# pierre-borie/Benlsip.jl

Hardware: AMD Instinct MI355X
Metric: PCG subproblems/sec + achieved HBM GB/s, dense m=65536 n=4096 fp64 (higher is better)
Workload: dtype f64

## Files before the change

benlsip.jl_amd/csrc/bh_api.hip:

```cpp
#include "../../include/benlsip_hip.h"
#include "bh_cauchy_plan.h"
#include "bh_free_image_plan.h"
#include "bh_gram_ingest_plan.h"
#include "bh_kernels.hip.h"
#include "bh_launch_ahead.h"
#include "bh_options.h"
#include "bh_pcg_plan.h"
#include "bh_step_chain_plan.h"

#include <dlfcn.h>
#include <fcntl.h>
#include <rccl/rccl.h>
#include <sched.h>
#include <sys/mman.h>
#include <unistd.h>

#include <algorithm>
#include <atomic>
#include <chrono>
#include <cmath>
#include <cstdio>
#include <cstdlib>
#include <cstring>
#include <array>
#include <initializer_list>
#include <string>
#include <thread>
#include <tuple>
#include <vector>

using namespace bh;

static uint64_t g_kernel_launches = 0;
static uint64_t g_mask_epoch = 0;
#undef hipLaunchKernelGGL
#define hipLaunchKernelGGL(kernelName, ...) do { ++g_kernel_launches; hipLaunchKernelGGLInternal((kernelName), __VA_ARGS__); } while (0)

namespace {

struct CgWorkspace {
    int64_t n_pad = 0;
    double *w = nullptr, *r = nullptr, *v = nullptr, *p = nullptr, *Hp = nullptr, *g = nullptr, *wl = nullptr, *wu = nullptr;
    double *x = nullptr, *s = nullptr, *xlow = nullptr, *xupp = nullptr;
    double* hw = nullptr;
    double* hwc = nullptr;
    double *p2 = nullptr, *gpart = nullptr, *rvpart = nullptr;
    double *r2 = nullptr, *hpx = nullptr, *hpx_tail = nullptr;
    double* slab = nullptr;
    double* scalars = nullptr;
    CgState* d_state = nullptr;
    volatile unsigned long long* h_mirror = nullptr;
    unsigned long long* d_mirror = nullptr;
    unsigned tag = 0;
    unsigned long long* d_reroute = nullptr;
    unsigned long long reroute_seq = 0;
    double* d_trace = nullptr;
    int64_t trace_cap = 0;
};

struct PeerShm {
    std::atomic<int> arrive;
    std::atomic<int> generation;
    int failed;
    hipIpcMemHandle_t handle[kMaxPeers];
};
struct PeerComm {
    bool active = false;
    bool broken = false;
    void* inbox = nullptr;
    size_t inbox_bytes = 0;
    void* peer_base[kMaxPeers] = {};
    volatile unsigned long long* h_err = nullptr;
    PeerShm* shm = nullptr;
    PeerArgs args{};
};
constexpr int64_t kPeerCap = 1 << 16;
constexpr int kPeerBlkCap = (int)(kPeerCap / (2 * kPeerBlockChunks));
constexpr size_t kPeerSlotBytes = (size_t)2 * kMaxPeers * kPeerCap * sizeof(double);
constexpr size_t kPeerFlagBytes = (size_t)2 * kMaxPeers * kPeerBlkCap * sizeof(unsigned long long);
constexpr size_t kPeerScalBytes = kPeerFlagBytes;

struct AsyncUpload {
    std::thread worker;
    int32_t rc = BH_OK;
    std::string detail;
    hipStream_t s_copy = nullptr, s_xpose = nullptr;
    double* staging[2] = {nullptr, nullptr};
    hipEvent_t copied[2] = {nullptr, nullptr}, freed[2] = {nullptr, nullptr};
    size_t staging_bytes = 0;
    int64_t chunk_cols = 0;
    bool gram = false;
    double gram_mu = 0.0;
    GramIngestPlan gram_plan{};
    hipStream_t s_gram = nullptr;
    double* gram_part = nullptr;
    int64_t gram_part_doubles = 0;
    bool resources() const { return s_copy != nullptr; }
};

struct Ctx : Options {
    bool init = false;
    int device = -1;
    int flags = 0;
    int n_cu = 0;
    hipStream_t own_stream = nullptr;
    hipStream_t stream = nullptr;
    std::string detail;
    StepNotes notes;
    void* rccl_lib = nullptr;
    ncclComm_t comm = nullptr;
    int rank = 0, nranks = 1;
    ncclResult_t (*p_ncclGetUniqueId)(ncclUniqueId*) = nullptr;
    ncclResult_t (*p_ncclCommInitRank)(ncclComm_t*, int, ncclUniqueId, int) = nullptr;
    ncclResult_t (*p_ncclCommDestroy)(ncclComm_t) = nullptr;
    ncclResult_t (*p_ncclAllReduce)(const void*, void*, size_t, ncclDataType_t, ncclRedOp_t, ncclComm_t, hipStream_t) = nullptr;
    const char* (*p_ncclGetErrorString)(ncclResult_t) = nullptr;
    PeerComm peer;
    int comm_path = 0;
    CgWorkspace cg;
    double* scratch_dev = nullptr;
    struct PooledImage { double* ptr; int64_t doubles; };
    std::vector<PooledImage> image_pool;
    int64_t image_pool_hits = 0;
    AsyncUpload* upload_cache = nullptr;
    int64_t h2d_bytes = 0, d2h_bytes = 0, h2d_calls = 0, d2h_calls = 0;
    volatile unsigned long long* mbox_h = nullptr;
    unsigned long long* mbox_d = nullptr;
    unsigned long long mbox_seq = 0;
    double* rbuf = nullptr;
    int64_t rbuf_cap = 0;
    int live_hess = 0;
    bool reform_vlds_attr_set = false;
    bool vlds_attr_set = false;
    bool cgp_vlds_attr_set = false;
    bool trsm_lds_granted = false;
    size_t trsv_lds_granted = 0;
};

// ... 223 lines not shown
    double* gpart = nullptr;
    int gram_slabs = 1;
    int64_t gram_slab_rows = 0;
    bool G_valid = false;
    double G_mu = 0.0;
    int64_t gram_builds = 0;
    double* geq = nullptr;
    int64_t geq_doubles = 0;
    double* Jf = nullptr;
    int64_t Jf_doubles = 0;
    int* fi_map = nullptr;
    int* fi_ops = nullptr;
    std::vector<int32_t> fi_ops_h;
    FreeImageBook fi;
    uint64_t fi_epoch = 0;
    double* Af = nullptr;
    int64_t Af_doubles = 0;
    uint64_t af_epoch = 0;
    double call_bytes = 0.0;
    double timed_bytes = 0.0;
    int64_t timed_n = 0;
};

struct bh_proj {
    int64_t mA = 0, n = 0, ldA = 0;
    double* Ad = nullptr;
    int nfix = 0, mpp = 0;
    bool active_set = false;
    int* fixrank = nullptr;
    int* fixidx = nullptr;
    double* L = nullptr;
    int64_t L_cap = 0;
    bool have_L = false;
    double* M = nullptr;
    double* Lr = nullptr;
    int* info = nullptr;
    double* tpart = nullptr;
    double* W = nullptr;
    bool linv_valid = false;
    int last_cauchy_form = -1;
    int last_cauchy_launches = 0;
    int last_cauchy_passes = 0;
    bool reduced = false;
    bool M_valid = false;
    std::vector<uint64_t> last_chunks;
    int* newidx = nullptr;
    int* counts = nullptr;
    unsigned long long* chunks_dev = nullptr;
    double* tw = nullptr;
    double* rpad = nullptr;
    double* vtmp = nullptr;
    uint64_t mask_epoch = 0;
};

namespace {

int32_t ensure_cg_workspace(int64_t n_pad, int64_t trace_cap) {
    CgWorkspace& c = g_ctx.cg;
    if (c.n_pad < n_pad) {
        double** vecs[] = {&c.w, &c.r, &c.v, &c.p, &c.Hp, &c.s, &c.x, &c.xlow, &c.xupp, &c.g, &c.wl, &c.wu, &c.hw, &c.hwc, &c.p2, &c.gpart, &c.rvpart,
                           &c.r2, &c.hpx, &c.hpx_tail};
        constexpr int NV = 20;
        dev_free(c.slab);
        c.slab = nullptr;
        g_ctx.notes.workspace_gone();
        BH_TRY(dev_alloc(&c.slab, NV * n_pad + 8));
        BH_HIP(hipMemsetAsync(c.slab, 0, (size_t)(NV * n_pad + 8) * sizeof(double), g_ctx.stream));
        for (int i = 0; i < NV; ++i) *vecs[i] = c.slab + (int64_t)i * n_pad;
        c.scalars = c.slab + NV * n_pad;
        c.n_pad = n_pad;
    }
    if (!c.d_state) {
        BH_TRY(dev_alloc(&c.d_state, 1));
        BH_HIP(hipMemsetAsync(c.d_state, 0, sizeof(CgState), g_ctx.stream));
        void* hp = nullptr;
        BH_HIP(hipHostMalloc(&hp, 64, hipHostMallocMapped | hipHostMallocCoherent));
        memset(hp, 0, 64);
        c.h_mirror = reinterpret_cast<volatile unsigned long long*>(hp);
        void* dp = nullptr;
        BH_HIP(hipHostGetDevicePointer(&dp, hp, 0));
        c.d_mirror = reinterpret_cast<unsigned long long*>(dp);
    }
    if (!c.d_reroute) {
        BH_TRY(dev_alloc(&c.d_reroute, 1));
        BH_HIP(hipMemsetAsync(c.d_reroute, 0, sizeof(unsigned long long), g_ctx.stream));
    }
    if (trace_cap > c.trace_cap) {
        dev_free(c.d_trace);
        c.d_trace = nullptr;
        BH_TRY(dev_alloc(&c.d_trace, 4 * trace_cap));
        c.trace_cap = trace_cap;
    }
    return BH_OK;
}

int32_t check_peer_error();
int32_t hess_ready(bh_hess* H);

int32_t wait_mirror(CgWorkspace& c, unsigned tag, int target, MirrorWord* out, int iter_target = 0) {
    const auto t0 = std::chrono::steady_clock::now();
    unsigned long long spins = 0;
    auto reached = [&](unsigned long long w, MirrorWord* m) {
        if (((w >> 48) & 0xffffu) != (tag & 0xffffu)) return false;
        m->status = (int)((w >> 44) & 0xf);
        m->done = (int)((w >> 40) & 0xf);
        m->iter = (int)((w >> 20) & 0xfffff);
        m->n_hmul = (int)(w & 0xfffff);
        return m->done != 0 || m->n_hmul >= target || (iter_target > 0 && m->iter >= iter_target);
    };
    while (true) {
        if (reached(*c.h_mirror, out)) return BH_OK;
        __builtin_ia32_pause();
        if ((++spins & 0xffff) == 0) {
            if (g_ctx.peer.active && *g_ctx.peer.h_err != 0ull) return check_peer_error();
            hipError_t q = hipStreamQuery(g_ctx.stream);
            if (q != hipSuccess && q != hipErrorNotReady) return fail(BH_ERR_HIP, std::string("CG loop: ") + hipGetErrorString(q));
            if (q == hipSuccess) {
                MirrorWord m2{};
                if (!reached(*c.h_mirror, &m2)) return fail(BH_ERR_HIP, "internal: stream drained but the loop state did not reach the launch target");
                continue;
            }
            if (std::chrono::steady_clock::now() - t0 > std::chrono::seconds(120))
                return fail(BH_ERR_HIP, "CG loop: no progress for 120 s", false);
        }
    }
}

bool comm_active() { return g_ctx.comm != nullptr || g_ctx.peer.active; }
bool use_peer_path() { return g_ctx.peer.active && (g_ctx.comm_path == 1 || g_ctx.comm == nullptr); }

int32_t allreduce_inplace(double* buf, int64_t count, bh_hess* H, const CgState* state = nullptr) {
    if (!comm_active() || count <= 0) return BH_OK;
    if (use_peer_path()) {
        for (int64_t off = 0; off < count; off += kPeerCap) {
            const int nch = (int)((std::min(kPeerCap, count - off) + 1) / 2);
            hipLaunchKernelGGL(reduce_exchange_kernel, dim3((nch + kPeerBlockChunks - 1) / kPeerBlockChunks), dim3(256), 0, g_ctx.stream,
                               (const double*)nullptr, (int64_t)0, nch, 0, buf + off, state, g_ctx.peer.args);
        }
        BH_HIP(hipGetLastError());
    } else {
        BH_NCCL(g_ctx.p_ncclAllReduce(buf, buf, (size_t)count, ncclDouble, ncclSum, g_ctx.comm, g_ctx.stream));
    }
    if (H) H->stats.n_allreduce += 1;
    return BH_OK;
}

int32_t check_peer_error() {
    if (g_ctx.peer.active && g_ctx.peer.h_err != nullptr && *g_ctx.peer.h_err != 0ull)
        return fail(BH_ERR_RCCL, "peer-buffer all-reduce: a rank did not arrive within the timeout (exchange #" +
                                     std::to_string(*g_ctx.peer.h_err) + "); results are invalid", false);
    return BH_OK;
}

int32_t reduce_slabs(bh_hess* H, int grid, double* z_out, const CgState* state) {
    const int nblk = (H->nchunks + kPeerBlockChunks - 1) / kPeerBlockChunks;
    if (use_peer_path() && nblk <= kPeerBlkCap) {
        hipLaunchKernelGGL(reduce_exchange_kernel, dim3(nblk), dim3(256), 0, g_ctx.stream, (const double*)H->partials, H->ld, H->nchunks,
                           grid, z_out, state, g_ctx.peer.args);
        BH_HIP(hipGetLastError());
        H->stats.n_allreduce += 1;
        return BH_OK;
    }
    hipLaunchKernelGGL(reduce_partials_kernel, dim3(nblk), dim3(256), 0, g_ctx.stream, H->partials, H->ld, H->nchunks, grid, z_out, state);
    BH_HIP(hipGetLastError());
    return allreduce_inplace(z_out, H->n, H, state);
}

constexpr int kPanelChunks = 2048;
// ... 1769 lines not shown
    in.hw_wanted = hw_wanted; in.hw_free_part_ok = hw_wanted && hw_free_part_ok; in.atol_f2b_positive = atol_f2b > 0; in.allow_free_image = allow_free_image;
    in.free_image_eq = g_ctx.opt_free_image_eq;
    p.sel = pcg_select(in);
    const int batch = launch_batch_size(H);
    const bool rccl_path = comm_active() && !use_peer_path();
    int cold = std::min(batch, rccl_path ? 1 : 2);
    p.sched.max_units = max_iter; p.sched.batch = batch; p.sched.off = 0; p.sched.look_first = true;
    p.sched.await_iter = false; p.sched.lock_step = true;
    p.pbuf[0] = c.p; p.pbuf[1] = c.p2;
    if (p.sel.shape == PCG_FUSED) {
        p.nrows = p.gram ? H->ld : H->d + H->q_eff;
        pcg_fused_geometry(p, H->nchunks, (int)n);
        p.vv_off = (int)(n_pad / 4);
        p.rvbuf[0] = c.rvpart; p.rvbuf[1] = c.rvpart + n_pad / 2;
        p.sched.await_iter = true; p.sched.lock_step = p.sel.rccl_gen;
        cold = p.sel.rccl_gen ? 1 : std::min(batch, 2);
    } else if (p.sel.shape == PCG_RCCL_BOX) {
        p.nrows = H->d + H->q_eff;
        p.cfg = rs_cfg; p.grid = grid_for(rs_cfg, p.nrows); p.nblk = (H->nchunks + 15) / 16;
        p.rbuf[0] = c.r; p.rbuf[1] = c.r2;
        p.gbuf[0] = H->sq_partials + H->g_cap; p.gbuf[1] = H->sq_partials + 2 * (int64_t)H->g_cap;
        cold = 1;
    }
    p.sched.first = launch_ahead_first(H->last_n_hmul, cold);
    return p;
}

static void pcg_use_free_image(PcgRun& r) {
    bh_hess* H = r.H; CgWorkspace& c = r.c;
    const FreeImageBook& b = H->fi;
    r.fi_use = true;
    r.og = c.x; r.owl = c.xlow; r.owu = c.xupp; r.ow = c.s;
    r.ofix = nullptr;
    if (r.hw != nullptr) r.hw = c.hwc;
    r.on = (int)b.nfree; r.onch = (int)(round_up(b.nfree, 16) / 2);
    r.old = b.ldf;
    pcg_fused_geometry(r.plan, r.onch, r.on);
    H->call_bytes = free_image_bytes(H);
    c.reroute_seq += 1;
}

static void pcg_compact_proj_args(ProjArgs& pa, const PcgRun& r) {
    pa.A = r.H->Af; pa.ldA = r.old; pa.n = r.on; pa.nfix = 0; pa.fixrank = nullptr; pa.nch_pad = r.onch;
}

static int32_t pcg_fused_stream(PcgRun& r, int j) {
    bh_hess* H = r.H; CgWorkspace& c = r.c; const PcgPlan& p = r.plan;
    RowStreamArgs ra = rs_args(H, p.nrows, nullptr);
    ra.partials = H->partials;
    if (p.gram) { ra.J = H->G; ra.d_rows = p.nrows; ra.mu = 1.0; ra.partials = nullptr; ra.t_out = c.Hp; }
    if (r.fi_use) { ra.J = H->Jf; ra.ld = r.old; ra.nchunks = r.onch; }
    if (p.sel.fuse_gen) { ra.v = c.p; ra.negate = 0; }
    else { ra.v = r.og; ra.negate = 1; ra.negmask = r.ofix; }
    CgFuse& f = ra.cf;
    f.st = c.d_state; f.j = j; f.n = r.on; f.max_iter = p.max_iter; f.init_done = p.sel.gen_linv ? 2 : p.sel.fuse_gen ? 1 : 0; f.vv_off = p.vv_off;
    f.vvec = c.v; f.p_old = p.pbuf[(j - 1) & 1]; f.p_new = p.pbuf[j & 1];
    f.rvpart = p.rvbuf[(j - 1) & 1]; f.nrv = p.nrv;
    f.w = r.ow; f.wl = r.owl; f.wu = r.owu;
    if (r.fi_use) { f.reroute = c.d_reroute; f.reroute_seq = c.reroute_seq; }
    f.sqpart = H->sq_partials; f.gpart = H->sq_partials + H->g_cap;
    f.kappa2 = r.a.kappa2; f.atol_f2b = r.a.atol_f2b;
    f.trace = r.a.trace; f.trace_cap = r.a.trace_cap; f.mirror = r.a.mirror; f.tag = r.a.tag;
    int slot = -1;
    const bool expect_stop = j == r.expect_stop_at || j > p.max_iter || (r.expect_stop_at == 0 && j > 1);
    BH_TRY(profile_begin(H, j - 1, &slot));
    if (p.gram) launch_gram_cg(p.cfg, ra, p.grid, r.s, expect_stop);
    else launch_row_stream_cgp(p.cfg, ra, p.grid, r.s, expect_stop);
    if (slot >= 0) BH_HIP(hipEventRecord(H->ev[2 * slot + 1], r.s));
    return BH_OK;
}

static int32_t pcg_fused_update(PcgRun& r, int j) {
    bh_hess* H = r.H; bh_proj* P = r.P; CgWorkspace& c = r.c; const PcgPlan& p = r.plan; hipStream_t s = r.s;
    const int nblk = p.nblk, grid = p.grid;
    CgUpdArgs u{};
    u.st = c.d_state; u.j = j; u.partials = H->partials; u.ld = r.old; u.nchunks = r.onch; u.G = grid; u.Gs = grid; u.Gq = grid;
    u.sqpart = H->sq_partials; u.gpart = H->sq_partials + H->g_cap; u.rvpart_in = p.rvbuf[(j - 1) & 1]; u.rvpart_out = p.rvbuf[j & 1]; u.nrv = p.nrv;
    u.p = p.pbuf[j & 1]; u.w = r.ow; u.hw = r.hw; u.r = c.r; u.g = r.og; u.v = c.v; u.fixrank = r.ofix;
    if (r.fi_use) { u.map = H->fi_map; u.w_full = r.wp; u.reroute = c.d_reroute; u.reroute_seq = c.reroute_seq; }
    u.n = r.on; u.atol_neg = r.a.atol_neg; u.trace = r.a.trace; u.trace_cap = r.a.trace_cap; u.mirror = r.a.mirror; u.tag = r.a.tag;
    if (p.gram) { u.partials = c.Hp; u.Gs = 1; }
    if (!p.sel.fuse_gen) {
        if (p.sel.peer_fused) hipLaunchKernelGGL((cg_reduce_update_kernel<false, true>), dim3(nblk), dim3(256), 0, s, u, g_ctx.peer.args);
        else hipLaunchKernelGGL((cg_reduce_update_kernel<false, false>), dim3(nblk), dim3(256), 0, s, u, PeerArgs{});
        return BH_OK;
    }
    if (p.sel.rccl_gen) {
        const int n_pad = r.a.n_pad;
        hipLaunchKernelGGL(reduce_partials_sq_kernel, dim3(nblk), dim3(256), 0, s, (const double*)H->partials, H->ld, H->nchunks, grid,
                           c.hpx, (const double*)H->sq_partials, n_pad, (const CgState*)c.d_state, j);
        BH_HIP(hipGetLastError());
        BH_TRY(allreduce_inplace(c.hpx, (int64_t)n_pad + 2, H));
        u.partials = c.hpx; u.Gs = 1; u.sqpart = c.hpx + n_pad; u.Gq = 1;
    }
    u.A = P->Ad; u.ldA = P->ldA; u.mA = (int)P->mA; u.tpart = P->tpart; u.init_in_memory = p.sel.gen_linv ? 0 : 1;
    if (r.fi_use) { u.A = H->Af; u.ldA = r.old; }
    if (r.fi_use) hipLaunchKernelGGL(cg_reduce_update_compact_kernel, dim3(nblk), dim3(256), 0, s, u);
    else if (p.sel.peer_fused) hipLaunchKernelGGL((cg_reduce_update_kernel<true, true>), dim3(nblk), dim3(256), 0, s, u, g_ctx.peer.args);
    else hipLaunchKernelGGL((cg_reduce_update_kernel<true, false>), dim3(nblk), dim3(256), 0, s, u, PeerArgs{});
    ProjArgs pa = proj_args(P, c.d_state, true);
    pa.tpart = P->tpart; pa.tpart_nblk = nblk; pa.rvpart = p.rvbuf[j & 1]; pa.fused_j = j;
    if (p.sel.gen_linv) {
        pa.W = P->W; pa.nch_pad = r.onch; pa.Mgram = p.sel.linv_refine ? P->M : nullptr;
        if (r.fi_use) pcg_compact_proj_args(pa, r);
        hipLaunchKernelGGL((proj_apply_linv_kernel<false>), dim3((unsigned)p.nrv), dim3(256), 0, s, pa, (const double*)c.r, c.v);
        return BH_OK;
    }
    hipLaunchKernelGGL(trsv_small_kernel, dim3(1), dim3(256), 0, s, pa);
    hipLaunchKernelGGL((proj_left_mul_tr_kernel<true, 4>), dim3((p.nch_v + 63) / 64), dim3(256), 0, s, pa, (const double*)c.r, c.v);
    return BH_OK;
}

static int32_t pcg_fused_first(PcgRun& r) {
    bh_hess* H = r.H; bh_proj* P = r.P; CgWorkspace& c = r.c; const PcgPlan& p = r.plan; hipStream_t s = r.s;
    if (r.fi_use) {
        FreeGatherArgs ga{};
        ga.g = r.a.g; ga.wl = r.a.wl; ga.wu = r.a.wu; ga.fixrank = P->fixrank; ga.map = H->fi_map;
        ga.gc = c.x; ga.wlc = c.xlow; ga.wuc = c.xupp; ga.wc = c.s; ga.w = r.wp;
        ga.n = r.a.n; ga.n_pad = r.a.n_pad; ga.nfree = r.on;
        ga.reroute = c.d_reroute; ga.seq = c.reroute_seq; ga.mirror = r.a.mirror; ga.tag = r.a.tag;
        hipLaunchKernelGGL(free_image_gather_kernel, dim3((unsigned)((r.a.n_pad + 255) / 256)), dim3(256), 0, s, ga);
    }
    if (p.sel.gen_linv) {
        if (!P->linv_valid) {
            hipLaunchKernelGGL(tri_inv_small_kernel, dim3(1), dim3(256), 0, s, (const double*)P->Lr, (int)P->mA, P->W);
            P->linv_valid = true;
        }
        ProjArgs pa = proj_args(P, nullptr, true);
        if (r.fi_use) pcg_compact_proj_args(pa, r);
        hipLaunchKernelGGL(proj_left_mul_kernel, dim3((unsigned)P->mA), dim3(256), 0, s, pa, r.og);
        pa.tpart = P->tw; pa.tpart_nblk = 1; pa.rvpart = p.rvbuf[0]; pa.vvpart = p.rvbuf[0] + p.vv_off; pa.p_out = c.p;
        pa.W = P->W; pa.nch_pad = r.onch; pa.Mgram = p.sel.linv_refine ? P->M : nullptr; pa.fused_j = 0;
        hipLaunchKernelGGL((proj_apply_linv_kernel<true>), dim3((unsigned)p.nrv), dim3(256), 0, s, pa, r.og, c.v);
    } else if (p.sel.fuse_gen) {
        hipLaunchKernelGGL((cg_init_kernel<false>), dim3(1), dim3(CG_T), 0, s, r.a);
        BH_TRY(launch_project(P, c.r, c.v, c.d_state));
        hipLaunchKernelGGL(cg_init_finish_kernel, dim3(1), dim3(CG_T), 0, s, r.a);
    }
    return pcg_fused_stream(r, 1);
}

static int32_t pcg_fused_unit(PcgRun& r, int index) {
    BH_TRY(pcg_fused_update(r, index + 1));
    BH_TRY(pcg_fused_stream(r, index + 2));
    BH_HIP(hipGetLastError());
    return BH_OK;
}

static int32_t pcg_rccl_box_stream(PcgRun& r, int j) {
    bh_hess* H = r.H; CgWorkspace& c = r.c; const PcgPlan& p = r.plan; const CgArgs& a = r.a;
    RowStreamArgs ra = rs_args(H, p.nrows, nullptr);
    ra.partials = H->partials;
    ra.v = a.g; ra.negate = 1; ra.negmask = a.fixrank;
    CgFuse& f = ra.cf;
    f.st = c.d_state; f.j = j; f.n = a.n; f.max_iter = p.max_iter; f.init_done = 0;
    f.p_old = p.pbuf[(j - 1) & 1]; f.p_new = p.pbuf[j & 1];
    f.r_old = p.rbuf[(j - 1) & 1]; f.r_new = p.rbuf[j & 1];
    f.gpart_in = p.gbuf[(j - 1) & 1]; f.gpart = p.gbuf[j & 1];
    f.w_rw = r.wp; f.w = r.wp; f.hw = r.hw; f.g = a.g; f.fixrank = a.fixrank;
    f.wl = a.wl; f.wu = a.wu;
    f.sqpart = H->sq_partials;
    f.Hp = c.hpx; f.sq_index = a.n_pad;
    f.kappa2 = a.kappa2; f.atol_f2b = a.atol_f2b; f.atol_neg = a.atol_neg;
    f.trace = a.trace; f.trace_cap = a.trace_cap; f.mirror = a.mirror; f.tag = a.tag;
    int slot = -1;
    BH_TRY(profile_begin(H, j - 1, &slot));
    launch_row_stream_cgp3(p.cfg, ra, p.grid, r.s);
// ... 28 lines not shown
    bh_hess* H = r.H; CgWorkspace& c = r.c;
    if (r.plan.sel.fold_init && index == 0) {
        BH_TRY(launch_hmul(H, r.a.g, c.Hp, nullptr, index, true, r.a.fixrank));
        launch_cg_first_step(r.a, r.s);
        return BH_OK;
    }
    BH_TRY(launch_hmul(H, c.p, c.Hp, c.d_state, index));
    if (r.P->mA == 0) {
        launch_cg_step<0>(r.a, r.s);
    } else {
        launch_cg_step<1>(r.a, r.s);
        BH_TRY(launch_project(r.P, c.r, c.v, c.d_state));
        launch_cg_step<2>(r.a, r.s);
    }
    return BH_OK;
}

static int32_t pcg_launch_first(PcgRun& r) {
    switch (r.plan.sel.shape) {
        case PCG_FUSED: return pcg_fused_first(r);
        case PCG_RCCL_BOX: return pcg_rccl_box_stream(r, 1);
        default: return pcg_separate_first(r);
    }
}
static int32_t pcg_launch_unit(PcgRun& r, int index) {
    switch (r.plan.sel.shape) {
        case PCG_FUSED: return pcg_fused_unit(r, index);
        case PCG_RCCL_BOX: return pcg_rccl_box_unit(r, index);
        default: return pcg_separate_unit(r, index);
    }
}

static int32_t pcg_run(bh_hess* H, bh_proj* P, const double* gp, const double* wlp, const double* wup, double* wp, bool w_in_ws,
                       double kappa2, double atol_negcurv, double atol_f2b, int64_t trace_cap, PcgFin* fin_out, double* hw = nullptr,
                       bool g_pad_zeroed = false ,
                       bool allow_free_image = true ,
                       bool hw_free_part_ok = false ) {
    const int64_t n = H->n, n_pad = H->ld;
    const int64_t max_iter64 = 2 * (n - P->mA - P->nfix);
    if (max_iter64 < 0) return fail(BH_ERR_PRECONDITION, "n - mA - count(fixvars) < 0");
    if (max_iter64 >= 0xfffff) return fail(BH_ERR_UNSUPPORTED, "2*(n - mA - count(fixvars)) exceeds the 20-bit iteration counters of the progress word");
    CgWorkspace& c = g_ctx.cg;
    H->ev_pending.clear();
    g_ctx.notes.cg_loop_begins(hw != nullptr);
    H->call_bytes = hmul_bytes(H);

    PcgRun run{H, P, c, g_ctx.stream};
    CgArgs& a = run.a;
    a.st = c.d_state; a.w = wp; a.r = c.r; a.v = c.v; a.p = c.p; a.Hp = c.Hp; a.g = gp; a.wl = wlp; a.wu = wup;
    a.fixrank = P->nfix > 0 ? P->fixrank : nullptr;
    a.n = (int)n; a.n_pad = (int)n_pad; a.w_in_ws = w_in_ws ? 1 : 0; a.max_iter = (int)max_iter64; a.kappa2 = kappa2; a.atol_neg = atol_negcurv; a.atol_f2b = atol_f2b;
    a.trace = trace_cap > 0 ? c.d_trace : nullptr; a.trace_cap = (int)std::min<int64_t>(trace_cap, 0x7fffffff);
    a.mirror = c.d_mirror; a.tag = next_mirror_tag(c);
    a.hw = hw;
    run.wp = wp; run.hw = hw;
    run.og = gp; run.owl = wlp; run.owu = wup; run.ow = wp; run.ofix = a.fixrank;
    run.on = (int)n; run.onch = H->nchunks; run.old = H->ld;
    run.expect_stop_at = H->last_n_hmul > 0 ? H->last_n_hmul + 1 : 0;

    run.plan = pcg_make_plan(H, P, a.max_iter, gp == c.g || n == n_pad, hw != nullptr, hw_free_part_ok, atol_f2b, allow_free_image);
    const PcgSelection& sel = run.plan.sel;
    if (sel.shape != PCG_SEPARATE) BH_TRY(hess_ready(H));
    if (sel.shape == PCG_FUSED && run.plan.gram) BH_TRY(ensure_gram(H));
    H->stats.cg_kernels = sel.cg_kernels;
    if (sel.shape != PCG_SEPARATE || sel.fold_init) BH_TRY(zero_staged_g_padding(c, gp, n, n_pad, g_pad_zeroed));
    bool fi_use = false, fi_earns = false;
    if (sel.free_image_eligible) BH_TRY(free_image_prepare(H, P, &fi_use, &fi_earns));
    if (fi_use && P->mA > 0) {
        BH_TRY(free_image_prepare_lineq(H, P, &fi_use));
        if (!fi_use) H->fi.served -= 1;
    }
    if (fi_use) pcg_use_free_image(run);

    BH_TRY(pcg_launch_first(run));
    MirrorWord mw{};
    BH_TRY(launch_ahead(run.plan.sched, [&](int index) { return pcg_launch_unit(run, index); },
                        [&](int n_hmul_target, int iter_target, MirrorWord* m) { return wait_mirror(c, a.tag, n_hmul_target, m, iter_target); }, &mw));
    if (!mw.done) return fail(BH_ERR_HIP, "internal: CG loop did not terminate");
    if (fi_use && mw.status == kCgReroute) {
        H->fi.served -= 1;
        return pcg_run(H, P, gp, wlp, wup, wp, w_in_ws, kappa2, atol_negcurv, atol_f2b, trace_cap, fin_out, hw, g_pad_zeroed, false);
    }
    if (fi_earns) H->fi.credit += free_image_saving(mw.n_hmul, P->nfix, n);
    const bool results_final = sel.shape == PCG_FUSED && !sel.rccl_gen &&
                               (mw.status == BH_CG_SOLVED || mw.status == BH_CG_MAX_ITER_REACHED || mw.status == BH_CG_NONE);
    pcg_fin_fill(fin_out, mw, a.tag, results_final);
    fin_out->compact = fi_use;
    if (sel.peer_fused) H->stats.n_allreduce += mw.n_hmul;
    return BH_OK;
}

static void read_tie_words(bh_hess* H) {
    const unsigned long long tw = g_ctx.cg.h_mirror[1], mb = g_ctx.cg.h_mirror[2];
    H->margin_kind = (int)((tw >> 48) & 0xf); H->tie_flags = (int)((tw >> 40) & 0xff);
    H->tie_first = (int)((tw >> 20) & 0xfffff); H->margin_at = (int)(tw & 0xfffff);
    memcpy(&H->min_margin, &mb, sizeof(double));
    H->tie_read = true;
}

static int32_t pcg_finish(bh_hess* H, const PcgFin& fin, bool drained = true) {
    if (!fin.done) return fail(BH_ERR_HIP, "internal: CG loop did not terminate");
    H->stats.n_pcg += 1;
    H->last_n_hmul = fin.n_hmul;
    H->tie_tag = fin.tag;
    H->tie_read = false;
    if (drained) read_tie_words(H);
    H->stats.n_hmul += fin.n_hmul;
    H->stats.n_cg_iter += fin.iter - 1;
    H->stats.n_proj += fin.iter;
    if (!H->ev_pending.empty()) {
        for (size_t i = 0; i < H->ev_pending.size(); ++i) {
            if (H->ev_pending[i] >= fin.n_hmul) continue;
            float ms = 0.f;
            if (hipEventElapsedTime(&ms, H->ev[2 * i], H->ev[2 * i + 1]) == hipSuccess) {
                H->stats.hmul_ms += ms;
                H->stats.hmul_timed += 1;
                H->timed_bytes += H->call_bytes;
                H->timed_n += 1;
            }
        }
        if (H->timed_n > 0) H->stats.bytes_per_hmul = H->timed_bytes / (double)H->timed_n;
        H->ev_pending.clear();
    }
    return BH_OK;
}

static int32_t pcg_impl(bh_hess* H, bh_proj* P, const double* g_minor, const double* w_l, const double* w_u, double kappa2,
                        double atol_negcurv, double atol_f2b, double* w_out, int32_t* status, int32_t* iters, double* trace,
                        int64_t trace_cap, int32_t* n_hmul_out, bool dev) {
    BH_REQUIRE_INIT();
    if (!H) return fail(BH_ERR_INVALID_ARG, "NULL bh_hess");
    BH_TRY(check_proj_ready(P));
    if (!g_minor || !w_l || !w_u || !w_out) return fail(BH_ERR_INVALID_ARG, "NULL vector argument");
    if (H->n != P->n) return fail(BH_ERR_SHAPE, "H.n != lincons.n");
    if (trace == nullptr) trace_cap = 0;
    if (trace_cap < 0) return fail(BH_ERR_INVALID_ARG, "negative trace_cap");
    const int64_t n = H->n;
    BH_TRY(ensure_cg_workspace(H->ld, trace_cap));
    CgWorkspace& c = g_ctx.cg;
    auto aligned16 = [](const void* q) { return (reinterpret_cast<uintptr_t>(q) & 15u) == 0; };
    const bool in_place = dev && (n % 2 == 0) && aligned16(g_minor) && aligned16(w_l) && aligned16(w_u) && aligned16(w_out) &&
                          (!comm_active() || n == H->ld);
    const double *gp = g_minor, *wlp = w_l, *wup = w_u;
    double* wp = w_out;
    if (!in_place) {
        if (!dev) {
            BH_TRY(stage_vecs(c.g, {g_minor, w_l, w_u}, n, c.n_pad));
        } else {
            BH_TRY(stage_vec(c.g, g_minor, n, true));
            BH_TRY(stage_vec(c.wl, w_l, n, true));
            BH_TRY(stage_vec(c.wu, w_u, n, true));
        }
        gp = c.g; wlp = c.wl; wup = c.wu; wp = c.w;
    }
    PcgFin fin{};
    BH_TRY(pcg_run(H, P, gp, wlp, wup, wp, !in_place, kappa2, atol_negcurv, atol_f2b, trace_cap, &fin, nullptr, !dev));
    if (!in_place) BH_TRY(fetch_vec(w_out, c.w, n, dev));
    if (trace_cap > 0) count_d2h((size_t)4 * trace_cap * sizeof(double));
    if (trace_cap > 0) note_dma();
    if (trace_cap > 0) BH_HIP(hipMemcpyAsync(trace, c.d_trace, (size_t)4 * trace_cap * sizeof(double), hipMemcpyDeviceToHost, g_ctx.stream));
    const bool drain = g_ctx.opt_final_sync || !(in_place && trace_cap == 0 && fin.results_final);
    if (drain) BH_TRY(sync_flush());
    BH_TRY(pcg_finish(H, fin, drain));
    if (status) *status = fin.status;
    if (iters) *iters = fin.iter;
    if (n_hmul_out) *n_hmul_out = fin.n_hmul;
    return BH_OK;
}
// ... 1053 lines not shown
```

benlsip.jl_amd/csrc/bh_cgfuse.hip.h:

```cpp
#pragma once
#include <hip/hip_runtime.h>
#include <stdint.h>
#include "bh_reduce.hip.h"
#include "bh_cg.hip.h"
#include "bh_comm.hip.h"

namespace bh {

struct CgUpdArgs {
    CgState* st;
    int j;
    const double* partials; int64_t ld; int nchunks; int G;
    int Gs, Gq;
    const double* sqpart;
    const double* gpart;
    const double* rvpart_in;
    double* rvpart_out;
    int nrv;
    const double* p;
    double* w; double* hw;
    double* r; const double* g;
    double* v;
    const int* fixrank;
    int n;
    double atol_neg;
    double* trace; int trace_cap;
    unsigned long long* mirror; unsigned tag;
    const double* A; int64_t ldA; int mA;
    double* tpart;
    int init_in_memory;
    const int* map; double* w_full;
    const unsigned long long* reroute; unsigned long long reroute_seq;
};

template <bool GEN, bool PEER>
__global__ __launch_bounds__(256) void cg_reduce_update_kernel(CgUpdArgs a, PeerArgs pa) {
    constexpr bool SCAT = !GEN;
#include "bh_cgfuse_body.hip.h"
}

__global__ __launch_bounds__(256) void cg_reduce_update_compact_kernel(CgUpdArgs a) {
    constexpr bool GEN = true, PEER = false, SCAT = true;
    const PeerArgs pa{};
#include "bh_cgfuse_body.hip.h"
}

}
```

benlsip.jl_amd/csrc/bh_cgfuse_body.hip.h:

```cpp
    CgState* st = a.st;
    if (st->stop_at != 0 && a.j > st->stop_at) return;
    if (a.reroute != nullptr && *a.reroute == a.reroute_seq) return;
    __shared__ double2 sm[16][17];
    __shared__ double rvs[16];
    __shared__ double2 rsm[16];
    const int tid = threadIdx.x, cl = tid & 15, rl = tid >> 4;
    const int c = blockIdx.x * 16 + cl;
    const bool valid = c < a.nchunks;
    const int64_t ld2 = a.ld >> 1;
    const double QNAN = __longlong_as_double(0x7ff8000000000000ll);

    const bool upd = (rl == 0) && valid;
    const bool from_g = (a.j == 1 && !a.init_in_memory);
    double2 pk = make_double2(0.0, 0.0), wk = pk, hwk = pk, rk = pk;
    int2 fr = make_int2(-1, -1);
    if (upd) {
        pk = reinterpret_cast<const double2*>(a.p)[c];
        if (from_g) {
            rk = reinterpret_cast<const double2*>(a.g)[c];
        } else {
            rk = reinterpret_cast<const double2*>(a.r)[c];
            wk = reinterpret_cast<const double2*>(a.w)[c];
            if (a.hw != nullptr) hwk = reinterpret_cast<const double2*>(a.hw)[c];
        }
    }
    TieRegs tr;
    tr.load(st);
    const int max_iter = st->max_iter;
    const double rtv_state = st->rtv;
    LaneBatch<8> b_sq, b_gp, b_rv;
    b_sq.issue(a.sqpart, a.Gq);
    b_gp.issue(a.gpart, a.G);
    b_rv.issue(a.rvpart_in, a.nrv);
    const double2* P2 = reinterpret_cast<const double2*>(a.partials);
    const int cc = min(c, a.nchunks - 1);
    SlabBatch sb;
    sb.issue(P2, ld2, cc, rl, a.Gs);
    double2 arow[4];
    if (GEN) {
        const double2* A2 = reinterpret_cast<const double2*>(a.A);
        const int64_t ldA2 = a.ldA >> 1;
#pragma unroll
        for (int k = 0; k < 4; ++k) arow[k] = A2[(int64_t)min(rl + 16 * k, a.mA - 1) * ldA2 + cc];
    }
    int2 mp = make_int2(-1, -1);
    if (SCAT && upd && a.map != nullptr) mp = reinterpret_cast<const int2*>(a.map)[c];
    if (upd && a.fixrank != nullptr) fr = reinterpret_cast<const int2*>(a.fixrank)[c];

    const double2 acc = sb.fold(P2, ld2, cc, rl, a.Gs);
    sm[rl][cl] = acc;

    double pHp = wave_sum(b_sq.fold_sum(a.sqpart, a.Gq));
    if (PEER) {
        __shared__ int s_timeout;
        __shared__ double2 xs[kMaxPeers][16];
        __shared__ double ps[kMaxPeers];
        if (tid == 0) s_timeout = 0;
        __syncthreads();
        if (rl == 0) {
            double2 t = sm[0][cl];
#pragma unroll
            for (int q = 1; q < 16; ++q) { t.x += sm[q][cl].x; t.y += sm[q][cl].y; }
            sm[15][cl] = t;
        }
        __syncthreads();
        const double2 mine = sm[15][cl];
        const unsigned long long seq = *pa.seq;
        const int par = (int)(seq & 1ull);
        const int64_t slot = ((int64_t)par * kMaxPeers + pa.rank) * pa.cap;
        const int64_t fidx = ((int64_t)par * kMaxPeers + pa.rank) * pa.nblk_cap + blockIdx.x;
        if (rl < pa.nranks && valid) sys_store_f64x2(pa.slots[rl] + slot + 2 * (int64_t)c, mine);
        if (rl < pa.nranks && cl == 0) __hip_atomic_store(pa.scal[rl] + fidx, pHp, __ATOMIC_RELAXED, __HIP_MEMORY_SCOPE_SYSTEM);
        asm volatile("s_waitcnt vmcnt(0)" ::: "memory");
        __syncthreads();
        if (rl < pa.nranks && cl == 0) __hip_atomic_store(pa.flags[rl] + fidx, seq, __ATOMIC_RELAXED, __HIP_MEMORY_SCOPE_SYSTEM);
        if (rl < pa.nranks && cl == 0) {
            const unsigned long long* f = pa.flags[pa.rank] + ((int64_t)par * kMaxPeers + rl) * pa.nblk_cap + blockIdx.x;
            const unsigned long long t0 = wall_clock64();
            const bool dead = __hip_atomic_load(pa.dead, __ATOMIC_RELAXED, __HIP_MEMORY_SCOPE_AGENT) != 0u;
            if (dead) s_timeout = 1;
            while (!dead && __hip_atomic_load(f, __ATOMIC_RELAXED, __HIP_MEMORY_SCOPE_SYSTEM) != seq) {
                __builtin_amdgcn_s_sleep(8);
                if (wall_clock64() - t0 > pa.timeout_ticks) {
                    s_timeout = 1;
                    __hip_atomic_store(pa.err, seq, __ATOMIC_RELAXED, __HIP_MEMORY_SCOPE_SYSTEM);
                    __hip_atomic_store(pa.dead, 1u, __ATOMIC_RELAXED, __HIP_MEMORY_SCOPE_AGENT);
                    break;
                }
            }
        }
        asm volatile("" ::: "memory");
        __syncthreads();
        if (rl < pa.nranks) {
            double2 got = make_double2(0.0, 0.0);
            if (valid) got = sys_load_f64x2(pa.slots[pa.rank] + ((int64_t)par * kMaxPeers + rl) * pa.cap + 2 * (int64_t)c);
            xs[rl][cl] = got;
            if (cl == 0) ps[rl] = __hip_atomic_load(pa.scal[pa.rank] + ((int64_t)par * kMaxPeers + rl) * pa.nblk_cap + blockIdx.x,
                                                  __ATOMIC_RELAXED, __HIP_MEMORY_SCOPE_SYSTEM);
        }
        __syncthreads();
        double2 t = xs[0][cl];
        double ph = ps[0];
        for (int r = 1; r < pa.nranks; ++r) { t.x += xs[r][cl].x; t.y += xs[r][cl].y; ph += ps[r]; }
        if (s_timeout) { ph = __longlong_as_double(0x7ff8000000000000ll); }
        pHp = ph;
        __syncthreads();
        sm[rl][cl] = (rl == 0) ? t : make_double2(0.0, 0.0);
        if (tid == 0) {
            const unsigned done = atomicAdd(pa.arrive, 1u) + 1u;
            if (done == gridDim.x) { *pa.arrive = 0u; *pa.seq = seq + 1ull; }
        }
    }
    const double gamma = wave_min(b_gp.fold_min(a.gpart, a.G));
    const double rtv = (a.j == 1) ? rtv_state : wave_sum(b_rv.fold_sum(a.rvpart_in, a.nrv));
    int cont = 0, neg = 0, outside = 0;
    double step = 0.0, alpha = QNAN;
    bool add_w = true;
    if (pHp <= a.atol_neg) {
        neg = 1;
        if (fabs(pHp) > a.atol_neg) step = gamma;
        else add_w = false;
    } else {
        alpha = __ddiv_rn(rtv, pHp);
        outside = alpha > gamma;
        if (outside) step = gamma;
        else { step = alpha; cont = 1; }
    }
    __syncthreads();

    double rv_part = 0.0;
    if (rl == 0 && valid) {
        double2 hp = sm[0][cl];
#pragma unroll
        for (int q = 1; q < 16; ++q) { hp.x += sm[q][cl].x; hp.y += sm[q][cl].y; }
        const bool e0 = 2 * c < a.n, e1 = 2 * c + 1 < a.n;
        if (add_w) {
            wk.x = __dadd_rn(wk.x, __dmul_rn(step, pk.x));
            wk.y = __dadd_rn(wk.y, __dmul_rn(step, pk.y));
            hwk.x = __dadd_rn(hwk.x, __dmul_rn(step, hp.x));
            hwk.y = __dadd_rn(hwk.y, __dmul_rn(step, hp.y));
        }
        double2 vk = make_double2(0.0, 0.0);
        if (cont) {
            rk.x = __dadd_rn(rk.x, __dmul_rn(alpha, hp.x));
            rk.y = __dadd_rn(rk.y, __dmul_rn(alpha, hp.y));
            vk.x = (fr.x >= 0) ? 0.0 : rk.x;
            vk.y = (fr.y >= 0) ? 0.0 : rk.y;
        }
        if (!e0) { wk.x = 0.0; hwk.x = 0.0; rk.x = 0.0; vk.x = 0.0; }
        if (!e1) { wk.y = 0.0; hwk.y = 0.0; rk.y = 0.0; vk.y = 0.0; }
        if (cont && !GEN) rv_part = fma(rk.y, vk.y, rk.x * vk.x);
        if (add_w || a.j == 1) {
            reinterpret_cast<double2*>(a.w)[c] = wk;
            if (a.hw != nullptr) reinterpret_cast<double2*>(a.hw)[c] = hwk;
            if (SCAT && mp.x >= 0) a.w_full[mp.x] = wk.x;
            if (SCAT && mp.y >= 0) a.w_full[mp.y] = wk.y;
        }
        if (cont || a.j == 1) {
            reinterpret_cast<double2*>(a.r)[c] = rk;
            if (!GEN) reinterpret_cast<double2*>(a.v)[c] = vk;
        }
        if (GEN) rsm[cl] = vk;
    } else if (GEN && rl == 0) {
        rsm[cl] = make_double2(0.0, 0.0);
    }
    if (!GEN) {
        if (rl == 0) rvs[cl] = rv_part;
        __syncthreads();
        if (tid == 0) {
            double t = 0.0;
#pragma unroll
            for (int q = 0; q < 16; ++q) t += rvs[q];
            a.rvpart_out[blockIdx.x] = t;
        }
    } else {
        __syncthreads();
        if (cont) {
            const double2 rm = rsm[cl];
#pragma unroll
            for (int k = 0; k < 4; ++k) {
                const int i = rl + 16 * k;
                if (i < a.mA) {
                    double prod = valid ? fma(arow[k].y, rm.y, arow[k].x * rm.x) : 0.0;
                    prod = row16_sum(prod);
                    if (cl == 0) a.tpart[(int64_t)blockIdx.x * a.mA + i] = prod;
                }
            }
        }
    }

    if (blockIdx.x == 0 && tid == 0) {
        st->pHp = pHp; st->gamma = gamma; st->alpha = alpha; st->n_hmul = a.j; st->rtv = rtv;
        st->neg_curvature = neg; st->outside_region = outside; st->need_proj = 0; st->iter = a.j;
        tr.note_step_a(pHp, a.atol_neg, alpha, gamma, a.j);
        tr.store(st);
        if (a.trace != nullptr && a.j <= a.trace_cap) {
            double* row = a.trace + 4 * (int64_t)(a.j - 1);
            row[0] = pHp; row[1] = alpha; row[2] = (neg && !add_w) ? QNAN : gamma; row[3] = rtv;
        }
        int status = 4;
        if (!cont) {
            status = cg_status_of(0, outside, neg, a.j, max_iter);
            st->approx_solved = 0; st->done = 1; st->stop_at = a.j;
            st->status = status;
        }
        publish_word(a.mirror, a.tag, status, cont ? 0 : 1, a.j, a.j, tr);
    }
```

benlsip.jl_amd/csrc/bh_pcg_plan.h:

```cpp
#pragma once
#include <cstdint>

namespace bh {

enum PcgShape : int {
    PCG_SEPARATE = 0,
    PCG_FUSED = 1,
    PCG_RCCL_BOX = 2,
};

struct PcgSelectIn {
    int64_t mA;
    bool gram_handle;
    int64_t cg_fused, gram_cg_fused, linv_refine, fold_init;
    bool comm, peer_path;
    bool reduced;
    bool tpart, W, M_valid;
    bool lda_is_ld;
    bool rs_cfg_ok;
    bool cgp3_ok;
    bool peer_blocks_fit;
    bool iterates;
    bool g_padded;
    bool vectors_in_regs;
    bool hw_wanted;
    bool atol_f2b_positive;
    bool allow_free_image;
    bool hw_free_part_ok;
    int64_t free_image_eq;
};

struct PcgSelection {
    PcgShape shape;
    bool fuse_gen;
    bool gen_linv;
    bool linv_refine;
    bool peer_fused;
    bool rccl_gen;
    bool free_image_eligible;
    bool fold_init;
    int cg_kernels;
};

inline PcgSelection pcg_select(const PcgSelectIn& in) {
    PcgSelection o{};
    const bool box = in.mA == 0;
    const int64_t cg_fused = !in.gram_handle ? in.cg_fused : (in.gram_cg_fused != 0 && !in.comm) ? 1 : 0;
    const bool fuse_gen = !box && cg_fused >= 1 && in.reduced && in.mA <= 64 && in.tpart && in.lda_is_ld && (!in.gram_handle || in.W);
    const bool gen_linv = fuse_gen && cg_fused == 1 && in.W;
    const bool peer_fused = in.comm && in.peer_path && (box || fuse_gen) && in.peer_blocks_fit;
    const bool rccl_gen = in.comm && !in.peer_path && fuse_gen;
    const bool feasible = in.rs_cfg_ok && in.iterates && in.g_padded;
    if ((box || fuse_gen) && cg_fused != 0 && feasible && (!in.comm || peer_fused || rccl_gen)) {
        o.shape = PCG_FUSED;
        o.fuse_gen = fuse_gen; o.gen_linv = gen_linv; o.peer_fused = peer_fused; o.rccl_gen = rccl_gen;
        o.linv_refine = gen_linv && in.linv_refine != 0 && in.M_valid && in.mA >= 2;
        o.cg_kernels = (box ? 2 : gen_linv ? 3 : 4) + (rccl_gen ? 1 : 0);
        o.free_image_eligible = in.allow_free_image && box && !in.gram_handle && !in.comm && (!in.hw_wanted || in.hw_free_part_ok) &&
                                in.atol_f2b_positive;
        if (in.free_image_eq != 0 && gen_linv && !in.gram_handle && !in.comm && !in.hw_wanted && in.atol_f2b_positive && in.allow_free_image)
            o.free_image_eligible = true;
        return o;
    }
    if (!in.gram_handle && in.comm && !in.peer_path && box && in.cg_fused != 0 && feasible && in.cgp3_ok) {
        o.shape = PCG_RCCL_BOX;
        o.cg_kernels = 2;
        return o;
    }
    o.shape = PCG_SEPARATE;
    o.fold_init = box && in.vectors_in_regs && in.fold_init != 0 && feasible;
    return o;
}

}
```

Before: 1778.

## Decide CG stop verdict in last-arriving block of fused update kernel

```diff
diff --git a/benlsip.jl_amd/csrc/bh_api.hip b/benlsip.jl_amd/csrc/bh_api.hip
--- a/benlsip.jl_amd/csrc/bh_api.hip
+++ b/benlsip.jl_amd/csrc/bh_api.hip
@@ -54,6 +54,7 @@
     unsigned tag = 0;
     unsigned long long* d_reroute = nullptr;
     unsigned long long reroute_seq = 0;
+    unsigned* d_arrive = nullptr;
     double* d_trace = nullptr;
     int64_t trace_cap = 0;
 };
@@ -443,8 +444,9 @@
         c.d_mirror = reinterpret_cast<unsigned long long*>(dp);
     }
     if (!c.d_reroute) {
-        BH_TRY(dev_alloc(&c.d_reroute, 1));
-        BH_HIP(hipMemsetAsync(c.d_reroute, 0, sizeof(unsigned long long), g_ctx.stream));
+        BH_TRY(dev_alloc(&c.d_reroute, 16));
+        BH_HIP(hipMemsetAsync(c.d_reroute, 0, 16 * sizeof(unsigned long long), g_ctx.stream));
+        c.d_arrive = reinterpret_cast<unsigned*>(c.d_reroute + 8);
     }
     if (trace_cap > c.trace_cap) {
         dev_free(c.d_trace);
@@ -2380,7 +2382,10 @@
     if (p.gram) { u.partials = c.Hp; u.Gs = 1; }
     if (!p.sel.fuse_gen) {
         if (p.sel.peer_fused) hipLaunchKernelGGL((cg_reduce_update_kernel<false, true>), dim3(nblk), dim3(256), 0, s, u, g_ctx.peer.args);
-        else hipLaunchKernelGGL((cg_reduce_update_kernel<false, false>), dim3(nblk), dim3(256), 0, s, u, PeerArgs{});
+        else {
+            u.arrive = c.d_arrive; u.verdict = pcg_update_takes_verdict(j, r.expect_stop_at, p.max_iter, p.gram) ? 1 : 0;
+            hipLaunchKernelGGL((cg_reduce_update_kernel<false, false>), dim3(nblk), dim3(256), 0, s, u, PeerArgs{});
+        }
         return BH_OK;
     }
     if (p.sel.rccl_gen) {
@@ -2575,8 +2580,9 @@
         return pcg_run(H, P, gp, wlp, wup, wp, w_in_ws, kappa2, atol_negcurv, atol_f2b, trace_cap, fin_out, hw, g_pad_zeroed, false);
     }
     if (fi_earns) H->fi.credit += free_image_saving(mw.n_hmul, P->nfix, n);
+    const bool ticket = sel.shape == PCG_FUSED && !sel.fuse_gen && !sel.peer_fused;
     const bool results_final = sel.shape == PCG_FUSED && !sel.rccl_gen &&
-                               (mw.status == BH_CG_SOLVED || mw.status == BH_CG_MAX_ITER_REACHED || mw.status == BH_CG_NONE);
+                               (ticket || mw.status == BH_CG_SOLVED || mw.status == BH_CG_MAX_ITER_REACHED || mw.status == BH_CG_NONE);
     pcg_fin_fill(fin_out, mw, a.tag, results_final);
     fin_out->compact = fi_use;
     if (sel.peer_fused) H->stats.n_allreduce += mw.n_hmul;
diff --git a/benlsip.jl_amd/csrc/bh_cgfuse.hip.h b/benlsip.jl_amd/csrc/bh_cgfuse.hip.h
--- a/benlsip.jl_amd/csrc/bh_cgfuse.hip.h
+++ b/benlsip.jl_amd/csrc/bh_cgfuse.hip.h
@@ -31,6 +31,7 @@
     int init_in_memory;
     const int* map; double* w_full;
     const unsigned long long* reroute; unsigned long long reroute_seq;
+    unsigned* arrive; int verdict;
 };
 
 template <bool GEN, bool PEER>
diff --git a/benlsip.jl_amd/csrc/bh_cgfuse_body.hip.h b/benlsip.jl_amd/csrc/bh_cgfuse_body.hip.h
--- a/benlsip.jl_amd/csrc/bh_cgfuse_body.hip.h
+++ b/benlsip.jl_amd/csrc/bh_cgfuse_body.hip.h
@@ -28,6 +28,8 @@
     tr.load(st);
     const int max_iter = st->max_iter;
     const double rtv_state = st->rtv;
+    double tol_cg = 0.0;
+    if constexpr (!GEN && !PEER) tol_cg = st->tol_cg;
     LaneBatch<8> b_sq, b_gp, b_rv;
     b_sq.issue(a.sqpart, a.Gq);
     b_gp.issue(a.gpart, a.G);
@@ -189,14 +191,41 @@
         }
     }
 
-    if (blockIdx.x == 0 && tid == 0) {
+    bool commit = blockIdx.x == 0 && tid == 0;
+    bool vstop = false, vsolved = false;
+    double rtv_next = 0.0;
+    if constexpr (!GEN && !PEER) {
+        if (!cont || a.verdict) {
+            __shared__ int s_last;
+            asm volatile("s_waitcnt vmcnt(0)" ::: "memory");
+            __syncthreads();
+            if (tid == 0) {
+                __builtin_amdgcn_fence(__ATOMIC_RELEASE, "agent");
+                asm volatile("s_waitcnt vmcnt(0)" ::: "memory");
+                s_last = __hip_atomic_fetch_add(a.arrive, 1u, __ATOMIC_RELAXED, __HIP_MEMORY_SCOPE_AGENT) == gridDim.x - 1u;
+            }
+            __syncthreads();
+            if (!s_last || tid >= 64) return;
+            __builtin_amdgcn_fence(__ATOMIC_ACQUIRE, "agent");
+            commit = tid == 0;
+            if (commit) __hip_atomic_store(a.arrive, 0u, __ATOMIC_RELAXED, __HIP_MEMORY_SCOPE_AGENT);
+            if (cont) {
+                rtv_next = wave_fixed_sum(a.rvpart_out, (int)gridDim.x);
+                vsolved = fabs(rtv_next) < tol_cg;
+                vstop = vsolved || a.j + 1 > max_iter;
+            }
+        }
+    }
+    if (commit) {
         st->pHp = pHp; st->gamma = gamma; st->alpha = alpha; st->n_hmul = a.j; st->rtv = rtv;
         st->neg_curvature = neg; st->outside_region = outside; st->need_proj = 0; st->iter = a.j;
         tr.note_step_a(pHp, a.atol_neg, alpha, gamma, a.j);
+        if constexpr (!GEN && !PEER) { if (vstop) tr.note(TIE_TOL, rel_margin(fabs(rtv_next), tol_cg), a.j); }
         tr.store(st);
         if (a.trace != nullptr && a.j <= a.trace_cap) {
             double* row = a.trace + 4 * (int64_t)(a.j - 1);
             row[0] = pHp; row[1] = alpha; row[2] = (neg && !add_w) ? QNAN : gamma; row[3] = rtv;
+            if constexpr (!GEN && !PEER) { if (vstop) row[3] = rtv_next; }
         }
         int status = 4;
         if (!cont) {
@@ -204,5 +233,15 @@
             st->approx_solved = 0; st->done = 1; st->stop_at = a.j;
             st->status = status;
         }
+        if constexpr (!GEN && !PEER) {
+            if (vstop) {
+                status = cg_status_of(vsolved ? 1 : 0, 0, 0, a.j + 1, max_iter);
+                st->iter = a.j + 1; st->beta = __ddiv_rn(rtv_next, rtv); st->rtv = rtv_next; st->approx_solved = vsolved ? 1 : 0;
+                st->done = 1; st->stop_at = a.j;
+                st->status = status;
+                publish_word(a.mirror, a.tag, status, 1, a.j + 1, a.j, tr);
+                return;
+            }
+        }
         publish_word(a.mirror, a.tag, status, cont ? 0 : 1, a.j, a.j, tr);
     }
diff --git a/benlsip.jl_amd/csrc/bh_pcg_plan.h b/benlsip.jl_amd/csrc/bh_pcg_plan.h
--- a/benlsip.jl_amd/csrc/bh_pcg_plan.h
+++ b/benlsip.jl_amd/csrc/bh_pcg_plan.h
@@ -42,6 +42,11 @@
     int cg_kernels;
 };
 
+inline bool pcg_update_takes_verdict(int j, int expect_stop_at, int max_iter, bool gram_handle) {
+    if (gram_handle) return false;
+    return j + 1 == expect_stop_at || j == max_iter;
+}
+
 inline PcgSelection pcg_select(const PcgSelectIn& in) {
     PcgSelection o{};
     const bool box = in.mA == 0;
```

After: 1783 (median of 3 runs). Within noise of the previous version (+0.2%).
